# taaha-khan/2023-CompaCT-Image-Compression

Measured on AMD Instinct MI355X. Metric: MPixels/s encode+decode, 12-bit 512x512 CT batch, bytes-exact, higher is better.
Workload: dtype u16

## Files before the change

2023-compact-image-compression_amd/csrc/api.cpp:

```cpp
#include <dlfcn.h>
#include <unistd.h>
#include <zlib.h>

#include <atomic>
#include <chrono>
#include <condition_variable>
#include <functional>
#include <cstdarg>
#include <cstdio>
#include <cstdlib>
#include <cstring>
#include <map>
#include <mutex>
#include <string>
#include <thread>
#include <vector>

#include "../../include/compact_hip.h"
#include "cct_internal.h"
#include "host.h"
#include "handoff.h"

namespace cct {
bool gilbert_table(int width, int height, int32_t *out);
// ... 667 lines not shown
	dfl_bind(a, base, shape);
	a.tree_waves = (uint32_t)g_ctx.tree_waves;
	a.pos_mask = (g_ctx.compact_recs && mem_level == 8 && in_stride < ((size_t)1 << 22)) ? (1u << 22) - 1u : 0xFFFFFFFFu;
	const DevBuf &mr = E.z_ws[DFL_R_MATCH];
	if (dfl_uses_chains(strategy)) {
		if (E.z_mr_cleared != mr.p || E.z_mr_cleared_cap != mr.cap || E.z_gen_passes >= 16000u) {
			HIP_TRY(hipMemsetAsync(mr.p, 0, mr.cap, E.stream));
			HIP_TRY(hipMemsetAsync(E.z_ws[DFL_R_GEN].p, 0, 256, E.stream));
			E.z_mr_cleared = mr.p; E.z_mr_cleared_cap = mr.cap; E.z_gen_passes = 0;
		}
		E.z_gen_passes++;
	}
	a.out = (uint8_t *)E.z_out.p; a.out_stride = out_stride; a.out_sizes = (uint32_t *)E.z_outsizes.p;
	memcpy(a.header13, header13, 13);
	if (g_ctx.use_graph) {
		std::vector<uint8_t> key(sizeof(DeflateArgs) + 2 * sizeof(int));
		memcpy(key.data(), &a, sizeof(DeflateArgs));
		memcpy(key.data() + sizeof(DeflateArgs), &n, sizeof(int));
		const int fork_key = use_fork ? 1 : 0;
		memcpy(key.data() + sizeof(DeflateArgs) + sizeof(int), &fork_key, sizeof(int));
		EncSlot::ZGraph *zg = nullptr;
		for (auto &g : E.z_graphs) if (g.key == key) zg = &g;
		if (!zg) {
			const int crc = exclusive_section([&]() -> int {
				if (E.z_graphs.size() >= 4) {
					size_t old = 0;
					for (size_t i = 1; i < E.z_graphs.size(); i++) if (E.z_graphs[i].last_use < E.z_graphs[old].last_use) old = i;
					if (E.z_graphs[old].exec) (void)hipGraphExecDestroy(E.z_graphs[old].exec);
					if (E.z_graphs[old].graph) (void)hipGraphDestroy(E.z_graphs[old].graph);
					E.z_graphs.erase(E.z_graphs.begin() + (long)old);
				}
				EncSlot::ZGraph g;
				HIP_TRY(hipStreamBeginCapture(E.stream, hipStreamCaptureModeThreadLocal));
				hipError_t le = launch_deflate(a, n, E.stream, use_fork ? E.stream_side : nullptr, E.ev_fork);
				hipError_t ce = hipStreamEndCapture(E.stream, &g.graph);
				if (le != hipSuccess) { if (g.graph) (void)hipGraphDestroy(g.graph); return fail(CCT_E_DEVICE, "DEFLATE capture: %s", hipGetErrorString(le)); }
				HIP_TRY(ce);
				const hipError_t ie = hipGraphInstantiate(&g.exec, g.graph, nullptr, nullptr, 0);
				if (ie != hipSuccess) { (void)hipGraphDestroy(g.graph); return fail(CCT_E_DEVICE, "hipGraphInstantiate failed: %s", hipGetErrorString(ie)); }
				g.key = key;
				E.z_graphs.push_back(std::move(g));
				return CCT_OK;
			});
			if (crc) return crc;
			zg = &E.z_graphs.back();
		}
		zg->last_use = ++E.z_clock;
		HIP_TRY(hipGraphLaunch(zg->exec, E.stream));
		return CCT_OK;
	}
	HIP_TRY(launch_deflate(a, n, E.stream, use_fork ? E.stream_side : nullptr, E.ev_fork));
	return CCT_OK;
}

int decode_payload_locked(DecSlot &D, const uint8_t *d_payload, size_t stride, const uint32_t *d_sizes, int n, int width,
                          int height, int bs, int fractal, uint16_t *d_images, uint32_t *d_status, hipStream_t st)
{
	const int N = width * height, NB = N / bs;
	if (stride % 16 != 0) return fail(CCT_E_ARG, "payload stride must be a multiple of 16");
	if (n == 0) return CCT_OK;
	DecArgs a{};
	a.payload = d_payload; a.stride = stride; a.sizes = d_sizes;
	a.lut = nullptr;
	a.n_tiles = 0; a.n_orient = 0; a.width = width;
	if (fractal) {
		const ShapeTables *tb;
		int rc0 = get_tables(width, height, &tb);
		if (rc0) return rc0;
		a.lut = tb->d_lut;
		if (tb->tiled && g_ctx.use_tiles && !g_ctx.runtime_bs) {
			a.tile_org = tb->d_org; a.tile_orient = tb->d_orient; a.patterns = tb->d_pat;
			a.n_tiles = tb->n_tiles; a.n_orient = tb->n_orient;
		}
	}
	a.N = N; a.NB = NB; a.images = d_images; a.status = d_status;
	const size_t per = (size_t)n * NB, jper = (size_t)n * ((size_t)NB / 2 + 1);
	int rc;
	if ((rc = D.d_role.ensure(per))) return rc;
	if ((rc = D.d_slot.ensure(per * 4))) return rc;
	if ((rc = D.d_jord.ensure(jper * 4))) return rc;
	if ((rc = D.d_jval.ensure(jper))) return rc;
	a.ws_role = (uint8_t *)D.d_role.p; a.ws_slot = (uint32_t *)D.d_slot.p;
	a.ws_jord = (uint32_t *)D.d_jord.p; a.ws_jval = (uint8_t *)D.d_jval.p;
	a.pcache_steps = (int)(stride / ((size_t)g_ctx.wg_threads * DEC_SEG) + 2);
	if ((rc = D.d_pcache.ensure((size_t)n * a.pcache_steps * g_ctx.wg_threads * sizeof(uint2)))) return rc;
	a.ws_pcache = (uint2 *)D.d_pcache.p;
	const bool run_time = bs_run_time(bs, g_ctx.runtime_bs != 0);
	HIP_TRY(launch_decode(a, n, bs, g_ctx.wg_threads, st, run_time));
	g_ctx.last_dec_path = run_time ? 1 : 0;
	if (st != D.stream) {
		HIP_TRY(hipEventRecord(D.ev_ws, st));
		HIP_TRY(hipStreamWaitEvent(D.stream, D.ev_ws, 0));
	}
	return CCT_OK;
}

}
}

using namespace cct;

extern "C" {

int cct_version(void) { return CCT_ABI_VERSION; }
const char *cct_last_error(void) { return g_err; }

int cct_init(int device)
{
	std::lock_guard<std::mutex> lk(g_mu);
	return ensure_ctx(device);
}

int cct_shutdown(void)
{
	std::lock_guard<std::mutex> lk(g_mu);
	std::lock_guard<std::mutex> lk1(g_mu1);
	std::lock_guard<std::mutex> lkd0(g_mu_dec[0]);
	std::lock_guard<std::mutex> lkd1(g_mu_dec[1]);
	if (!g_ctx.ready || g_ctx.pid != getpid()) { reset_ctx(); return CCT_OK; }
	(void)hipSetDevice(g_ctx.device);
	(void)hipStreamSynchronize(g_ctx.stream);
	(void)hipStreamSynchronize(g_ctx.stream_dec);
	for (int k = 0; k < N_ENC_SLOTS; k++) {
		EncSlot &E = g_enc[k];
		if (E.stream) (void)hipStreamSynchronize(E.stream);
		if (E.stream_copy) (void)hipStreamSynchronize(E.stream_copy);
		for (auto &g : E.z_graphs) { if (g.exec) (void)hipGraphExecDestroy(g.exec); if (g.graph) (void)hipGraphDestroy(g.graph); }
		for (int i = 0; i < E.n_bufs; i++) E.all_bufs[i]->release();
		for (HandoffSet &S : E.sets) S.release();
		for (hipEvent_t e : E.ev_fork) if (e) (void)hipEventDestroy(e);
		E.ev_zlib.release();
		if (E.stream_copy) (void)hipStreamDestroy(E.stream_copy);
		if (E.stream_side) { (void)hipStreamSynchronize(E.stream_side); (void)hipStreamDestroy(E.stream_side); }
		if (k > 0 && E.stream) (void)hipStreamDestroy(E.stream);
	}
	comm_release();
	dicom_rle_release();
	jpegll_release();
	jpegls_release();
	j2k_release();
	tiff_release();
	if (g_gate) { (void)hipFree(g_gate); g_gate = nullptr; }
	for (auto &kv : g_ctx.luts) {
		ShapeTables &t = kv.second;
		void *ptrs[] = {t.d_lut, t.d_org, t.d_orient, t.d_pat, t.d_ptab, t.d_otab, t.d_ttab, t.d_htab};
		for (void *p : ptrs) if (p) (void)hipFree(p);
	}
	for (int k = 0; k < N_DEC_SLOTS; k++) {
		DecSlot &D = g_dec[k];
		if (D.stream) (void)hipStreamSynchronize(D.stream);
		D.release();
		if (k > 0 && D.stream) (void)hipStreamDestroy(D.stream);
	}
	(void)hipStreamDestroy(g_ctx.stream);
	(void)hipStreamDestroy(g_ctx.stream_dec);
	reset_ctx();
	return CCT_OK;
}

int cct_device_info(char *name, size_t name_cap, int *compute_units, uint64_t *hbm_bytes)
{
	std::lock_guard<std::mutex> lk(g_mu);
	int rc = ensure_ctx();
	if (rc) return rc;
	hipDeviceProp_t prop;
	HIP_TRY(hipGetDeviceProperties(&prop, g_ctx.device));
	if (name && name_cap) {
		char dn[256] = "";
// ... 1307 lines not shown
```

2023-compact-image-compression_amd/csrc/cct_internal.h:

```cpp
#pragma once
#include <stddef.h>
#include <stdint.h>
#include <string.h>

#include <vector>

#include <hip/hip_runtime.h>

#include "deflate_workspace.h"
#include "tuning.h"

namespace cct {

constexpr int ENC_CH = 8192;
constexpr int ENC_RING = 4;
constexpr int ENC_LIST_CAP = 1536;
constexpr int ENC_STG_BYTES = 2 * ENC_CH + ENC_CH / 8 + 64;
constexpr int ENC_MAX_LDS_ROLE = 48 * 1024;

constexpr uint8_t ROLE_PARTNER = 0xFF;

struct EncArgs {
	const uint16_t *images;
	const int32_t *lut;
	int N, NB;
	int eof;
	uint32_t flags;
	uint8_t *payload; size_t stride;
	uint32_t *sizes; uint32_t *status;
	uint8_t *ws_role;
	uint32_t *ws_lidx;
	uint64_t *ws_lmask;
	uint8_t *ws_lcur;
	uint32_t *stats;
	uint8_t *roles_out;
	uint32_t dbg_skip;
	int bs;
};
static_assert(sizeof(EncArgs) == 120, "EncArgs layout: bs must stay in the tail padding");

constexpr int TILE_MAX_TILES = 1024;
constexpr int TILE_MAX_ORIENT = 4;
struct TileEncArgs {
	EncArgs e;
	const uint32_t *tile_org;
	const uint8_t *tile_orient;
	const uint16_t *patterns;
	int n_orient, n_tiles, row_pitch;
};
size_t enc_tiles_lds_bytes(int NB, bool *role_in_lds);
hipError_t launch_encode_tiles(const TileEncArgs &ta, int n, hipStream_t s);

constexpr int STREAM_MAX_NB = 65536;
constexpr int STREAM_PAIR_REC = 80;
constexpr uint32_t CCT_ST_INTERNAL = 0x80000000u;
struct StreamTiles {
	uint32_t orgo[256];
	uint32_t last[TILE_MAX_ORIENT];
	uint32_t qorg[TILE_MAX_ORIENT];
};
constexpr int STREAM_TPG = 4;
struct StreamArgs {
	EncArgs e;
	StreamTiles tiles;
	const uint32_t *ptab;
	const uint32_t *htab;
	const uint32_t *otab;
	const uint32_t *ttab;
	int n_tiles, row_pitch, gps, tpg;
	int dbg;
	uint64_t *hand;
	uint32_t *ticket;
	uint64_t *spill_mask;
	uint16_t *spill_idx;
	uint8_t *pairrec;
};
inline size_t stream_ws_bytes(int n, int gps) { return ((size_t)n * gps * 32 + (size_t)n * 4 + 15) & ~(size_t)15; }
hipError_t launch_encode_stream(const StreamArgs &sa, int n, hipStream_t s);

size_t enc_lds_bytes(int NB, bool *role_in_lds);
inline bool bs_run_time(int bs, bool force) { return force || (bs & (bs - 1)) != 0; }

hipError_t launch_encode(const EncArgs &a, int n, int block_size, int threads, hipStream_t s, bool run_time);

constexpr int DEC_SEG = 16;
constexpr int DEC_JLIST_CAP = 2048;

struct DecArgs {
	const uint8_t *payload; size_t stride; const uint32_t *sizes;
	const int32_t *lut;
	int N, NB;
	uint16_t *images; uint32_t *status;
	uint8_t *ws_role;
	uint32_t *ws_slot;
	uint32_t *ws_jord;
	uint8_t *ws_jval;
	const uint32_t *tile_org; const uint8_t *tile_orient; const uint16_t *patterns;
	int n_tiles, n_orient, width;
	uint32_t bs_mul;
	uint2 *ws_pcache; int pcache_steps;
	uint16_t bs, bs_shift;
};
static_assert(sizeof(DecArgs) == 144, "DecArgs layout: the run-time block size fields must stay in padding");

inline void bs_divider(int d, uint32_t *mul, uint32_t *shift)
{
	uint32_t s = 0;
	while ((2u << s) <= (uint32_t)(d - 1)) s++;
	*shift = s;
	*mul = (uint32_t)((((uint64_t)1 << (32 + s)) + (uint64_t)d - 1) / (uint64_t)d);
}

hipError_t launch_decode(const DecArgs &a, int n, int block_size, int threads, hipStream_t s, bool run_time);

bool deflate_level_args(int level, DeflateArgs &a);
bool deflate_mem_level_args(int mem_level, DeflateArgs &a);
bool deflate_strategy_args(int level, int strategy, DeflateArgs &a);
hipError_t deflate_init_tables();
hipError_t launch_pack(const uint8_t *src, size_t stride, const uint32_t *sizes, int n, uint64_t *offsets, uint8_t *dst,
                       int exact, hipStream_t st);
hipError_t launch_deflate(const DeflateArgs &a, int n, hipStream_t st, hipStream_t side = nullptr,
                          const hipEvent_t *fork_join_events = nullptr);

hipError_t launch_png_filter(const uint16_t *d_img, int n, int rows, int cols, int shift, uint8_t *d_out, size_t out_stride,
                             hipStream_t st);
hipError_t launch_png_filter8(const void *d_img, int src_bits, int n, int rows, int cols, int lo, int hi, uint8_t *d_out,
                              size_t out_stride, hipStream_t st);
struct PngPackArgs {
	const uint8_t *src; size_t src_stride; uint32_t src_skip;
	const uint32_t *src_sizes;
	uint32_t chunk;
	uint8_t ihdr[25];
	uint8_t *out; size_t out_stride; uint32_t *out_sizes;
};
hipError_t launch_png_pack(const PngPackArgs &a, int n, uint32_t max_chunks, hipStream_t st);

struct PngChunk {
	uint64_t src;
	uint64_t dst;
	uint32_t len;
	uint32_t file;
};
constexpr uint32_t PNG_CHUNK_IDAT = 1u << 31;
constexpr uint32_t PNG_ST_CRC = 1u, PNG_ST_FILTER = 2u, PNG_ST_SKIP = 4u;
struct PngUnpackArgs {
	const uint8_t *files;
	const PngChunk *chunks;
	uint8_t *streams;
	uint32_t *status;
};
hipError_t launch_png_unpack(const PngUnpackArgs &a, uint32_t n_chunks, hipStream_t st);
struct PngUnfilterArgs {
	uint8_t *rows; size_t rows_stride;
	const uint32_t *row_sizes, *zstatus;
	uint32_t *status;
	const uint8_t *bpp;
	int nrows, cols, shift;
	uint16_t *images;
};
constexpr int PNG_UNFILTER_WAVES = 8;
hipError_t launch_png_unfilter(const PngUnfilterArgs &a, int n, int waves, hipStream_t st);

hipError_t launch_gate_bump(uint32_t *word, hipStream_t st);
hipError_t launch_gate_wait(const uint32_t *gate, uint32_t want_pass, uint32_t grace_us, uint32_t timeout_us, hipStream_t st);

struct InflateArgs {
	const uint8_t *in; uint64_t in_total;
	const uint64_t *offsets; int skip;
	uint8_t *out; size_t out_stride;
// ... 347 lines not shown
```

2023-compact-image-compression_amd/csrc/decode_kernels.hip:

```cpp
#include "cct_internal.h"
#include "wave_device.h"
#include "../../include/compact_hip.h"

namespace cct {
namespace {

struct SegStats {
	uint32_t exit_state;
	uint32_t npix;
	uint32_t njump;
	int32_t sdelta;
};

__device__ __forceinline__ int tok_delta_full(uint32_t b0, uint32_t b1)
{
	int x = (int)(((b0 << 8) | b1) & 0xFFFu);
	return x > 2048 ? x - 4096 : x;
}
__device__ __forceinline__ int tok_delta_short(uint32_t b0)
{
	int x = (int)(b0 & 0x7Fu);
	return x > 64 ? x - 128 : x;
}

__device__ __forceinline__ uint32_t seg_byte(const uint4 &w, uint32_t nxt, int i)
{
	const uint32_t word = (i < 4) ? w.x : (i < 8) ? w.y : (i < 12) ? w.z : (i < 16) ? w.w : nxt;
	return (word >> ((i & 3) * 8)) & 0xFFu;
}

struct SegMasks { uint32_t F, J, S, V; };

__device__ __forceinline__ uint32_t msb_nibble(uint32_t m) { return ((m >> 7) * 0x01020408u) >> 24; }

__device__ __forceinline__ SegMasks seg_masks(const uint4 &w, int nvalid)
{
	const uint32_t ws[4] = {w.x, w.y, w.z, w.w};
	SegMasks m{0, 0, 0, nvalid >= 16 ? 0xFFFFu : ((1u << max(nvalid, 0)) - 1u)};
#pragma unroll
	for (int k = 0; k < 4; k++) {
		const uint32_t x = ws[k];
		const uint32_t t = (x & 0xF0F0F0F0u) ^ 0xE0E0E0E0u;
		const uint32_t nz = (((t & 0x7F7F7F7Fu) + 0x7F7F7F7Fu) | t) & 0x80808080u;
		m.F |= msb_nibble(nz ^ 0x80808080u) << (4 * k);
		m.J |= msb_nibble(x & ~(x << 1) & 0x80808080u) << (4 * k);
		m.S |= msb_nibble(~x & 0x80808080u) << (4 * k);
	}
	m.F &= m.V; m.J &= m.V; m.S &= m.V;
	return m;
}

__device__ __forceinline__ void seg_structure(const SegMasks &m, uint32_t e, uint32_t &second, uint32_t &fulls)
{
	const uint32_t ODD = 0xAAAAAAAAu;
	const uint32_t pe = m.F & ~e;
	const uint32_t etc = (((pe << 1) | ODD) - pe) ^ ODD;
	second = (etc ^ (m.F | e)) & m.V;
	fulls = etc & m.F;
}

__device__ __forceinline__ SegStats seg_stats(const uint4 &w, uint32_t nxt, const SegMasks &m, int nvalid, uint32_t e)
{
	SegStats st{e, 0, 0, 0};
	if (nvalid <= 0) return st;
	uint32_t second, fulls;
	seg_structure(m, e, second, fulls);
	const uint32_t starts = m.V & ~second;
	st.exit_state = (fulls >> (nvalid - 1)) & 1u;
	st.njump = (uint32_t)__popc(starts & m.J);
	st.npix = (uint32_t)__popc(starts & ~m.J);
	const uint32_t sh = starts & m.S;
	const uint32_t ws[4] = {w.x, w.y, w.z, w.w};
	uint32_t sum = 0, big = 0;
#pragma unroll
	for (int k = 0; k < 4; k++) {
		const uint32_t sel = (((sh >> (4 * k)) & 15u) * 0x00204081u) & 0x01010101u;
		sum = __builtin_amdgcn_udot4(ws[k], sel, sum, false);
		big += (uint32_t)__popc(((((ws[k] & 0x7F7F7F7Fu) + 0x3F3F3F3Fu) & 0x80808080u) >> 7) & sel);
	}
	st.sdelta = (int32_t)sum - 128 * (int32_t)big;
	for (uint32_t f = fulls; f; f &= f - 1) {
		const int i = __ffs((int)f) - 1;
		st.sdelta += tok_delta_full(seg_byte(w, nxt, i), seg_byte(w, nxt, i + 1));
	}
	return st;
}

__device__ __forceinline__ uint32_t map_apply(uint32_t m, uint32_t s) { return (m >> s) & 1u; }
__device__ __forceinline__ uint32_t map_compose(uint32_t later, uint32_t earlier)
{
	return map_apply(later, map_apply(earlier, 0)) | (map_apply(later, map_apply(earlier, 1)) << 1);
}

struct Parse {
	uint32_t entry;
	uint32_t pix_base;
	int32_t val_base;
	uint32_t jump_base;
	SegStats st;
};

__device__ __forceinline__ Parse parse_step(const uint4 &w, uint32_t nxt, int nvalid,
                                           uint32_t *scratch, uint32_t &st_carry,
                                           uint32_t &npix_carry, int32_t &val_carry,
                                           uint32_t &njump_carry)
{
	const int lane = threadIdx.x & 63, wave = threadIdx.x >> 6, nw = blockDim.x >> 6;
	const SegMasks sm = seg_masks(w, nvalid);
	const SegStats s0 = seg_stats(w, nxt, sm, nvalid, 0);
	const SegStats s1 = seg_stats(w, nxt, sm, nvalid, 1);
	uint32_t m = s0.exit_state | (s1.exit_state << 1);
	m = map_compose(m, dpp_move<DPP_ROW_SHR1>(m, 2));
	m = map_compose(m, dpp_move<DPP_ROW_SHR2>(m, 2));
	m = map_compose(m, dpp_move<DPP_ROW_SHR4>(m, 2));
	m = map_compose(m, dpp_move<DPP_ROW_SHR8>(m, 2));
	m = map_compose(m, dpp_move<DPP_ROW_BCAST15, 0xA>(m, 2));
	m = map_compose(m, dpp_move<DPP_ROW_BCAST31, 0xC>(m, 2));
	const uint32_t excl = dpp_move<DPP_WAVE_SHR1>(m, 2);
	if (lane == 63) scratch[wave] = m;
	__syncthreads();
	uint32_t st_wave = st_carry, st_end = st_carry;
	for (int x = 0; x < nw; x++) {
		const uint32_t wm = scratch[x];
		if (x < wave) st_wave = map_apply(wm, st_wave);
		st_end = map_apply(wm, st_end);
	}
	Parse p;
	p.entry = map_apply(excl, st_wave);
	p.st = p.entry ? s1 : s0;
	const uint32_t ipj = wave_incl_scan(p.st.npix | (p.st.njump << 16));
	const uint32_t iv = wave_incl_scan((uint32_t)p.st.sdelta);
	const uint32_t ip = ipj & 0xFFFFu, ij = ipj >> 16;
	if (lane == 63) { scratch[16 + wave] = ipj; scratch[32 + wave] = iv; }
	__syncthreads();
	uint32_t bpj = 0, bv = 0, tpj = 0, tv = 0;
	for (int x = 0; x < nw; x++) {
		const uint32_t xp = scratch[16 + x], xv = scratch[32 + x];
		if (x < wave) { bpj += xp; bv += xv; }
		tpj += xp; tv += xv;
	}
	const uint32_t bp = bpj & 0xFFFFu, bj = bpj >> 16, tp = tpj & 0xFFFFu, tj = tpj >> 16;
	p.pix_base = npix_carry + bp + ip - p.st.npix;
	p.val_base = val_carry + (int32_t)(bv + iv - (uint32_t)p.st.sdelta);
	p.jump_base = njump_carry + bj + ij - p.st.njump;
	st_carry = st_end;
	npix_carry += tp;
	val_carry += (int32_t)tv;
	njump_carry += tj;
	return p;
}

template <int BS, bool TAB_LDS, bool TILED = false>
__global__ void __launch_bounds__(1024) decode_kernel(DecArgs a)
{
	static_assert(BS != 0 || !TILED, "the tiled variant exists for block size 16 only");
	extern __shared__ __attribute__((aligned(16))) uint8_t dyn_lds[];
	__shared__ uint32_t scratch[64];
	__shared__ uint32_t l_jord[DEC_JLIST_CAP];
	__shared__ uint8_t l_jval[DEC_JLIST_CAP];
	__shared__ uint32_t s_status;

	const int tid = threadIdx.x, T = blockDim.x;
	const int s = blockIdx.x;
	const int N = a.N, NB = a.NB;
	const uint8_t *P = a.payload + (size_t)s * a.stride;
	const uint32_t L = a.sizes[s];
	const uint32_t Lr = min((uint32_t)a.stride, L) > 0 ? min((uint32_t)a.stride, L) - 1u : 0u;
	const int32_t *lut = a.lut;
	uint16_t *out = a.images + (size_t)s * N;
	const uint32_t bs = BS ? (uint32_t)BS : (uint32_t)a.bs;
	auto bdiv = [&](uint32_t x) -> uint32_t { return BS ? x / (uint32_t)BS : __umulhi(x, a.bs_mul) >> a.bs_shift; };
	auto bmod = [&](uint32_t x) -> uint32_t { return BS ? x % (uint32_t)BS : x - bdiv(x) * bs; };
	typedef __attribute__((address_space(3))) uint8_t lds_u8;
	typedef __attribute__((address_space(3))) uint32_t lds_u32;
	lds_u32 *l_slot = (lds_u32 *)dyn_lds;
	lds_u8 *l_role = (lds_u8 *)(dyn_lds + (size_t)NB * 4);
	uint8_t *g_role = a.ws_role + (size_t)s * NB;
	uint32_t *g_slot = a.ws_slot + (size_t)s * NB;
	auto role_rd = [&](uint32_t b) -> uint32_t { return TAB_LDS ? (uint32_t)l_role[b] : (uint32_t)g_role[b]; };
	auto role_wr = [&](uint32_t b, uint32_t v) { if (TAB_LDS) l_role[b] = (uint8_t)v; else g_role[b] = (uint8_t)v; };
	auto slot_rd = [&](uint32_t i) -> uint32_t { return TAB_LDS ? l_slot[i] : g_slot[i]; };
	auto slot_wr = [&](uint32_t i, uint32_t v) { if (TAB_LDS) l_slot[i] = v; else g_slot[i] = v; };
	typedef __attribute__((address_space(3))) uint16_t lds_u16;
	constexpr uint32_t PAT_STRIDE = 4096 + 256;
	lds_u16 *l_pat = (lds_u16 *)(dyn_lds + (((size_t)NB * 5 + 15) & ~(size_t)15));
	lds_u32 *l_torg = (lds_u32 *)(l_pat + (TILED ? (size_t)a.n_orient * PAT_STRIDE : 0));
	lds_u8 *l_tori = (lds_u8 *)(l_torg + (TILED ? a.n_tiles : 0));
	if (TILED) {
		for (int i = tid; i < a.n_orient * 4096; i += T) {
			const uint32_t pv = a.patterns[i];
			const uint32_t dy = pv >> 7, dx = ((((pv >> 4) & 7u) ^ (dy & 7u)) << 3) | ((pv & 15u) >> 1);
			const uint32_t o = (uint32_t)i >> 12, p = (uint32_t)i & 4095u;
			l_pat[o * PAT_STRIDE + p + (p >> 4)] = (uint16_t)(dy * (uint32_t)a.width + dx);
		}
		for (int i = tid; i < a.n_tiles; i += T) { l_torg[i] = a.tile_org[i]; l_tori[i] = a.tile_orient[i]; }
	}
	auto raster_of = [&](uint32_t pos) -> uint32_t {
		if (TILED) {
			const uint32_t tile = pos >> 12;
			const uint32_t p = pos & 4095u;
			return l_torg[tile] + l_pat[(uint32_t)l_tori[tile] * PAT_STRIDE + p + (p >> 4)];
		}
		return lut ? (uint32_t)lut[pos] : pos;
	};
	const size_t jcap = (size_t)NB / 2 + 1;
	uint32_t *g_jord = a.ws_jord + (size_t)s * jcap;
	uint8_t *g_jval = a.ws_jval + (size_t)s * jcap;

#ifdef CCT_DEC_PROF
	long long tp[8]; int tpi = 0;
#define DEC_STAMP() do { if (tpi < 8) tp[tpi++] = clock64(); } while (0)
#else
#define DEC_STAMP() do {} while (0)
#endif
	DEC_STAMP();
	if (tid == 0) s_status = 0;
	for (int b = tid; b < NB; b += T) role_wr((uint32_t)b, 0);
	__syncthreads();
	DEC_STAMP();

	const uint32_t seg_max = (uint32_t)a.stride - 16u;
	auto load_seg = [&](uint32_t seg_start, uint4 &w, uint32_t &nxt) {
		w = *reinterpret_cast<const uint4 *>(P + min(seg_start, seg_max));
		nxt = P[min(seg_start + 16u, (uint32_t)a.stride - 1u)];
	};
	auto clip_seg = [&](uint32_t seg_start, uint4 &w, uint32_t &nxt, int &nvalid) {
		const bool inside = seg_start < Lr;
		nvalid = inside ? (int)min(16u, Lr - seg_start) : 0;
		if (!inside) w = make_uint4(0, 0, 0, 0);
		if (!(seg_start + 16u < Lr)) nxt = 0;
	};
	auto jset = [&](uint32_t k, uint32_t ord, uint32_t j) {
		if (k < DEC_JLIST_CAP) { l_jord[k] = ord; l_jval[k] = (uint8_t)j; }
		else if (k - DEC_JLIST_CAP < jcap) { g_jord[k - DEC_JLIST_CAP] = ord; g_jval[k - DEC_JLIST_CAP] = (uint8_t)j; }
	};

	uint32_t st_c = 0, npix_c = 0, nj_c = 0;
	int32_t val_c = 0;
	uint2 *pcache = a.ws_pcache + (size_t)s * a.pcache_steps * T;
	uint32_t nsteps = 0;
	uint4 wa_n; uint32_t nxta_n;
	load_seg((uint32_t)tid * DEC_SEG, wa_n, nxta_n);
	for (uint32_t base = 0; base < Lr && npix_c < (uint32_t)N; base += (uint32_t)T * DEC_SEG, nsteps++) {
		uint4 w = wa_n; uint32_t nxt = nxta_n; int nvalid;
		clip_seg(base + (uint32_t)tid * DEC_SEG, w, nxt, nvalid);
		load_seg(base + (uint32_t)(T + tid) * DEC_SEG, wa_n, nxta_n);
		const Parse p = parse_step(w, nxt, nvalid, scratch, st_c, npix_c, val_c, nj_c);
		asm volatile("" : "+v"(wa_n.x), "+v"(wa_n.y), "+v"(wa_n.z), "+v"(wa_n.w), "+v"(nxta_n) :: "memory");
		pcache[(size_t)nsteps * T + tid] = make_uint2(min(p.pix_base, 0x7FFFFFFFu) | (p.entry << 31), (uint32_t)p.val_base);
		if (p.st.njump) {
			const SegMasks sm = seg_masks(w, nvalid);
			uint32_t second, fulls;
			seg_structure(sm, p.entry, second, fulls);
			const uint32_t starts = sm.V & ~second, pix = starts & ~sm.J;
			uint32_t k = p.jump_base;
			for (uint32_t jm = starts & sm.J; jm; jm &= jm - 1, k++) {
				const int i = __ffs((int)jm) - 1;
				const uint32_t ord = p.pix_base + (uint32_t)__popc(pix & ((1u << i) - 1u));
				jset(k, ord, seg_byte(w, nxt, i) & 0x3Fu);
			}
		}
	}
	__syncthreads();
	DEC_STAMP();
	if (npix_c < (uint32_t)N && tid == 0) atomicOr(&s_status, CCT_ST_STREAM);

	if (tid < 64) {
		auto uni = [](uint32_t x) { return (uint32_t)__builtin_amdgcn_readfirstlane((int)x); };
		const uint32_t nj = uni(nj_c);
		uint32_t F = 0;
		uint64_t win = 0;
		uint32_t slots_done = 0;
		bool bad = false;
		auto fetch = [&](uint32_t k, uint32_t &ord, uint32_t &j) {
			ord = 0xFFFFFFFFu; j = 0;
			if (k < DEC_JLIST_CAP) { ord = l_jord[k]; j = l_jval[k]; }
			else if (k - DEC_JLIST_CAP < jcap) { ord = g_jord[k - DEC_JLIST_CAP]; j = g_jval[k - DEC_JLIST_CAP]; }
		};
		uint32_t ord_n = 0, j_n = 0;
		if (nj) fetch(0, ord_n, j_n);
		for (uint32_t k = 0; k < nj && !bad; k++) {
			if (k >= DEC_JLIST_CAP && k - DEC_JLIST_CAP >= jcap) { bad = true; break; }
			const uint32_t ord = uni(ord_n), j = uni(j_n);
			if (k + 1 < nj) fetch(k + 1, ord_n, j_n);
			if (ord >= (uint32_t)N) break;
			if (bmod(ord) != 0) { bad = true; break; }
			const uint32_t sslot = bdiv(ord);
			if (sslot < slots_done) { bad = true; break; }
			uint32_t remaining = sslot - slots_done;
			while (remaining) {
				if (win == 0) { F += remaining; remaining = 0; break; }
				const uint32_t o = (uint32_t)__ffsll((long long)win) - 1u;
				if (o >= remaining) { F += remaining; win >>= remaining; remaining = 0; }
				else { F += o + 1; win = (o + 1 >= 64u) ? 0ull : (win >> (o + 1)); remaining -= o; }
			}
			{ const uint64_t free_ = ~win; const uint32_t t = free_ ? (uint32_t)__builtin_ctzll(free_) : 64u; F += t; win = t >= 64u ? 0ull : win >> t; }
			const uint32_t Lb = F, pb = F + j;
			if (j == 0 || pb >= (uint32_t)NB || ((win >> j) & 1ull)) { bad = true; break; }
			if (tid == 0) { role_wr(Lb, j); role_wr(pb, ROLE_PARTNER); }
			win |= 1ull << j;
			F = Lb + 1;
			win >>= 1;
			slots_done = sslot + 2;
		}
		if (bad && tid == 0) atomicOr(&s_status, CCT_ST_STREAM);
	}
	__syncthreads();
	DEC_STAMP();

	{
		uint32_t slot_c = 0;
		for (int base = 0; base < NB; base += T) {
			const int b = base + tid;
			uint32_t r = ROLE_PARTNER, cnt = 0;
			if (b < NB) { r = role_rd((uint32_t)b); cnt = (r == ROLE_PARTNER) ? 0u : (r ? 2u : 1u); }
			const int lane = tid & 63, wave = tid >> 6, nw = T >> 6;
			const uint32_t inc = wave_incl_scan(cnt);
			if (lane == 63) scratch[wave] = inc;
			__syncthreads();
			uint32_t bs_ = 0, tot = 0;
			for (int x = 0; x < nw; x++) { const uint32_t v = scratch[x]; if (x < wave) bs_ += v; tot += v; }
			__syncthreads();
			const uint32_t sl = slot_c + bs_ + inc - cnt;
			if (cnt >= 1 && sl < (uint32_t)NB) slot_wr(sl, (uint32_t)b | (cnt == 2 ? (1u << 30) : 0u));
			if (cnt == 2 && sl + 1 < (uint32_t)NB) slot_wr(sl + 1, (uint32_t)b | (2u << 30));
			slot_c += tot;
		}
		if (slot_c != (uint32_t)NB && tid == 0) atomicOr(&s_status, CCT_ST_STREAM);
	}
	__syncthreads();
	DEC_STAMP();

	if (!(s_status & CCT_ST_STREAM)) {
		uint4 w_n; uint32_t nxt_n;
		load_seg((uint32_t)tid * DEC_SEG, w_n, nxt_n);
		uint2 pc_n = pcache[tid];
#ifdef CCT_DEC_PROF
		long long tb[4] = {0, 0, 0, 0}, tq = clock64();
#define DECB(j) do { const long long t_ = clock64(); tb[j] += t_ - tq; tq = t_; } while (0)
#else
#define DECB(j) do {} while (0)
#endif
		for (uint32_t k = 0; k < nsteps; k++) {
			const uint32_t seg_start = k * (uint32_t)T * DEC_SEG + (uint32_t)tid * DEC_SEG;
			uint4 w = w_n; uint32_t nxt = nxt_n; int nvalid;
			clip_seg(seg_start, w, nxt, nvalid);
			const uint2 pc = pc_n;
			load_seg(seg_start + (uint32_t)T * DEC_SEG, w_n, nxt_n);
			pc_n = pcache[(size_t)min(k + 1, nsteps - 1) * T + tid];
			Parse p;
			p.entry = pc.x >> 31; p.pix_base = pc.x & 0x7FFFFFFFu; p.val_base = (int32_t)pc.y;
			const SegMasks sm = seg_masks(w, nvalid);
			uint32_t second, fulls;
			seg_structure(sm, p.entry, second, fulls);
			uint32_t starts = sm.V & ~second, pix = starts & ~sm.J;
			uint32_t ord = p.pix_base;
			int32_t val = p.val_base;
			uint32_t flags = 0;
			const uint32_t room = ord < (uint32_t)N ? (uint32_t)N - ord : 0u;
			if ((uint32_t)__popc(pix) > room) {
				uint32_t keep = 0;
				if (room) {
					uint32_t pm = pix;
					for (uint32_t r = 1; r < room; r++) pm &= pm - 1;
					keep = (2u << (__ffs((int)pm) - 1)) - 1u;
				}
				starts &= keep; pix &= keep; fulls &= keep;
			}
			DECB(0);
			if (nvalid > 0 && ((fulls >> (nvalid - 1)) & 1u) && seg_start + (uint32_t)nvalid >= Lr) flags |= CCT_ST_STREAM;
			if (BS ? BS >= 16 : bs >= 16) {
				struct SlotInfo { uint32_t kind, pos0, pos1, org0, org1, idx0, idx1; };
				auto slot_info = [&](uint32_t sl) {
					SlotInfo si{0, 0, 0, 0, 0, 0, 0};
					const uint32_t ent = slot_rd(min(sl, (uint32_t)NB - 1u));
					const uint32_t blk0 = ent & 0x3FFFFFFFu; si.kind = ent >> 30;
					const uint32_t blk1 = si.kind ? blk0 + role_rd(blk0) : blk0;
					si.pos0 = blk0 * bs; si.pos1 = blk1 * bs;
					if (TILED) {
						const uint32_t t0 = si.pos0 >> 12, t1 = si.pos1 >> 12, b0 = si.pos0 & 4095u, b1 = si.pos1 & 4095u;
						si.org0 = l_torg[t0]; si.idx0 = (uint32_t)l_tori[t0] * PAT_STRIDE + b0 + (b0 >> 4);
						si.org1 = l_torg[t1]; si.idx1 = (uint32_t)l_tori[t1] * PAT_STRIDE + b1 + (b1 >> 4);
					}
					return si;
				};
				const uint32_t slA = bdiv(ord);
				const SlotInfo A = slot_info(slA), B = slot_info(slA + 1u);
				DECB(1);
				const uint32_t ws[5] = {w.x, w.y, w.z, w.w, nxt};
#pragma unroll
				for (int i = 0; i < 16; i++) {
					if (!((pix >> i) & 1u)) continue;
					const uint32_t c = (ws[i >> 2] >> (8 * (i & 3))) & 0xFFu;
					const uint32_t c1 = (ws[(i + 1) >> 2] >> (8 * ((i + 1) & 3))) & 0xFFu;
					val += ((sm.S >> i) & 1u) ? tok_delta_short(c) : ((fulls >> i) & 1u) ? tok_delta_full(c, c1) : 0;
					if ((uint32_t)val > 65535u) flags |= CCT_ST_OVERFLOW;
					const uint32_t sl = bdiv(ord), t = bmod(ord);
					const bool inA = sl == slA;
					const uint32_t kind = inA ? A.kind : B.kind;
					uint32_t odd = 0, off = t;
					if (kind) { const uint32_t mm = (kind - 1u) * bs + t; odd = mm & 1u; off = mm >> 1; }
					uint32_t ras;
					if (TILED) {
						const uint32_t org = inA ? (odd ? A.org1 : A.org0) : (odd ? B.org1 : B.org0);
						const uint32_t idx = inA ? (odd ? A.idx1 : A.idx0) : (odd ? B.idx1 : B.idx0);
						ras = org + l_pat[idx + off + (BS > 16 ? off >> 4 : 0u)];
					} else ras = raster_of((inA ? (odd ? A.pos1 : A.pos0) : (odd ? B.pos1 : B.pos0)) + off);
					out[ras] = (uint16_t)val;
					ord++;
				}
			} else {
				uint32_t cur_sl = 0xFFFFFFFFu, kind = 0, blk0 = 0, blk1 = 0;
				uint32_t org0 = 0, org1 = 0, pat0 = 0, pat1 = 0;
				for (uint32_t pm = pix; pm; pm &= pm - 1) {
					const int i = __ffs((int)pm) - 1;
					const uint32_t c = seg_byte(w, nxt, i);
					if ((sm.S >> i) & 1u) val += tok_delta_short(c);
					else if ((fulls >> i) & 1u) val += tok_delta_full(c, seg_byte(w, nxt, i + 1));
					if (val < 0 || val > 65535) flags |= CCT_ST_OVERFLOW;
					const uint32_t sl = bdiv(ord), t = bmod(ord);
					if (sl != cur_sl) {
						cur_sl = sl;
						const uint32_t ent = slot_rd(sl);
						blk0 = ent & 0x3FFFFFFFu; kind = ent >> 30;
						blk1 = kind ? blk0 + role_rd(blk0) : blk0;
						if (TILED) {
							const uint32_t t0 = (blk0 * bs) >> 12, t1 = (blk1 * bs) >> 12;
							org0 = l_torg[t0]; pat0 = (uint32_t)l_tori[t0] * PAT_STRIDE;
							org1 = l_torg[t1]; pat1 = (uint32_t)l_tori[t1] * PAT_STRIDE;
						}
					}
					uint32_t pos, odd = 0;
// ... 71 lines not shown
```

Baseline: 18410.

## Overlap jump-list replay with parsing using a dedicated wave in decode

The last wave of the decode workgroup no longer parses segments. It incrementally replays the jump list (role assignment) in chunks while the other waves parse, instead of one wave running the whole replay serially after the parse finishes. Parsing now computes only the exit-state map first and the segment stats once for the known entry state, rather than stats for both entry states. The cross-wave combines use DPP row scans and readlane instead of serial loops over scratch. The second pass is restructured to iterate over a flat segment index because the parse stride is now threads-64. The cost is one fewer parsing wave, so each workgroup needs more parse steps.

```diff
diff --git a/2023-compact-image-compression_amd/csrc/api.cpp b/2023-compact-image-compression_amd/csrc/api.cpp
--- a/2023-compact-image-compression_amd/csrc/api.cpp
+++ b/2023-compact-image-compression_amd/csrc/api.cpp
@@ -773,8 +773,9 @@
 	if ((rc = D.d_jval.ensure(jper))) return rc;
 	a.ws_role = (uint8_t *)D.d_role.p; a.ws_slot = (uint32_t *)D.d_slot.p;
 	a.ws_jord = (uint32_t *)D.d_jord.p; a.ws_jval = (uint8_t *)D.d_jval.p;
-	a.pcache_steps = (int)(stride / ((size_t)g_ctx.wg_threads * DEC_SEG) + 2);
-	if ((rc = D.d_pcache.ensure((size_t)n * a.pcache_steps * g_ctx.wg_threads * sizeof(uint2)))) return rc;
+	const size_t dec_tp = (size_t)dec_parse_lanes(g_ctx.wg_threads);
+	a.pcache_steps = (int)(stride / (dec_tp * DEC_SEG) + 2);
+	if ((rc = D.d_pcache.ensure((size_t)n * a.pcache_steps * dec_tp * sizeof(uint2)))) return rc;
 	a.ws_pcache = (uint2 *)D.d_pcache.p;
 	const bool run_time = bs_run_time(bs, g_ctx.runtime_bs != 0);
 	HIP_TRY(launch_decode(a, n, bs, g_ctx.wg_threads, st, run_time));
diff --git a/2023-compact-image-compression_amd/csrc/cct_internal.h b/2023-compact-image-compression_amd/csrc/cct_internal.h
--- a/2023-compact-image-compression_amd/csrc/cct_internal.h
+++ b/2023-compact-image-compression_amd/csrc/cct_internal.h
@@ -85,6 +85,7 @@
 
 constexpr int DEC_SEG = 16;
 constexpr int DEC_JLIST_CAP = 2048;
+constexpr int dec_parse_lanes(int threads) { return threads - 64; }
 
 struct DecArgs {
 	const uint8_t *payload; size_t stride; const uint32_t *sizes;
diff --git a/2023-compact-image-compression_amd/csrc/decode_arith.h b/2023-compact-image-compression_amd/csrc/decode_arith.h
--- /dev/null
+++ b/2023-compact-image-compression_amd/csrc/decode_arith.h
@@ -0,0 +1,140 @@
+#pragma once
+#include <stdint.h>
+
+#if defined(__HIP__)
+#include <hip/hip_runtime.h>
+#define CCT_HD __host__ __device__ __forceinline__
+#else
+#define CCT_HD inline
+#endif
+
+namespace cct {
+namespace {
+
+struct SegWords { uint32_t x, y, z, w; };
+
+CCT_HD int tok_delta_full(uint32_t b0, uint32_t b1)
+{
+	int x = (int)(((b0 << 8) | b1) & 0xFFFu);
+	return x > 2048 ? x - 4096 : x;
+}
+CCT_HD int tok_delta_short(uint32_t b0)
+{
+	int x = (int)(b0 & 0x7Fu);
+	return x > 64 ? x - 128 : x;
+}
+
+CCT_HD uint32_t seg_byte(const SegWords &w, uint32_t nxt, int i)
+{
+	const uint32_t word = (i < 4) ? w.x : (i < 8) ? w.y : (i < 12) ? w.z : (i < 16) ? w.w : nxt;
+	return (word >> ((i & 3) * 8)) & 0xFFu;
+}
+
+struct SegMasks { uint32_t F, J, S, V; };
+
+CCT_HD uint32_t msb_nibble(uint32_t m) { return ((m >> 7) * 0x01020408u) >> 24; }
+
+CCT_HD SegMasks seg_masks(const SegWords &w, int nvalid)
+{
+	const uint32_t ws[4] = {w.x, w.y, w.z, w.w};
+	SegMasks m{0, 0, 0, nvalid >= 16 ? 0xFFFFu : ((1u << (nvalid > 0 ? nvalid : 0)) - 1u)};
+#ifdef __HIP__
+#pragma unroll
+#endif
+	for (int k = 0; k < 4; k++) {
+		const uint32_t x = ws[k];
+		const uint32_t t = (x & 0xF0F0F0F0u) ^ 0xE0E0E0E0u;
+		const uint32_t nz = (((t & 0x7F7F7F7Fu) + 0x7F7F7F7Fu) | t) & 0x80808080u;
+		m.F |= msb_nibble(nz ^ 0x80808080u) << (4 * k);
+		m.J |= msb_nibble(x & ~(x << 1) & 0x80808080u) << (4 * k);
+		m.S |= msb_nibble(~x & 0x80808080u) << (4 * k);
+	}
+	m.F &= m.V; m.J &= m.V; m.S &= m.V;
+	return m;
+}
+
+CCT_HD void seg_structure(const SegMasks &m, uint32_t e, uint32_t &second, uint32_t &fulls)
+{
+	const uint32_t ODD = 0xAAAAAAAAu;
+	const uint32_t pe = m.F & ~e;
+	const uint32_t etc = (((pe << 1) | ODD) - pe) ^ ODD;
+	second = (etc ^ (m.F | e)) & m.V;
+	fulls = etc & m.F;
+}
+
+constexpr uint32_t MAP_IDENT = 2;
+CCT_HD uint32_t map_apply(uint32_t m, uint32_t s) { return (m >> s) & 1u; }
+CCT_HD uint32_t map_compose(uint32_t later, uint32_t earlier)
+{
+	return map_apply(later, map_apply(earlier, 0)) | (map_apply(later, map_apply(earlier, 1)) << 1);
+}
+
+CCT_HD uint32_t seg_exit_map(const SegMasks &m, int nvalid)
+{
+	if (nvalid <= 0) return MAP_IDENT;
+	uint32_t second, f0, f1;
+	seg_structure(m, 0, second, f0);
+	seg_structure(m, 1, second, f1);
+	return ((f0 >> (nvalid - 1)) & 1u) | (((f1 >> (nvalid - 1)) & 1u) << 1);
+}
+
+struct SegStats {
+	uint32_t exit_state;
+	uint32_t npix;
+	uint32_t njump;
+	int32_t sdelta;
+};
+
+CCT_HD uint32_t dot4_u8(uint32_t w, uint32_t sel, uint32_t acc)
+{
+#if defined(__HIP_DEVICE_COMPILE__)
+	return __builtin_amdgcn_udot4(w, sel, acc, false);
+#else
+	for (int b = 0; b < 4; b++) acc += ((w >> (8 * b)) & 0xFFu) * ((sel >> (8 * b)) & 0xFFu);
+	return acc;
+#endif
+}
+
+CCT_HD SegStats seg_stats(const SegWords &w, uint32_t nxt, const SegMasks &m, int nvalid, uint32_t e)
+{
+	SegStats st{e, 0, 0, 0};
+	if (nvalid <= 0) return st;
+	uint32_t second, fulls;
+	seg_structure(m, e, second, fulls);
+	const uint32_t starts = m.V & ~second;
+	st.exit_state = (fulls >> (nvalid - 1)) & 1u;
+	st.njump = (uint32_t)__builtin_popcount(starts & m.J);
+	st.npix = (uint32_t)__builtin_popcount(starts & ~m.J);
+	const uint32_t sh = starts & m.S;
+	const uint32_t ws[4] = {w.x, w.y, w.z, w.w};
+	uint32_t sum = 0, big = 0;
+#ifdef __HIP__
+#pragma unroll
+#endif
+	for (int k = 0; k < 4; k++) {
+		const uint32_t sel = (((sh >> (4 * k)) & 15u) * 0x00204081u) & 0x01010101u;
+		sum = dot4_u8(ws[k], sel, sum);
+		big += (uint32_t)__builtin_popcount(((((ws[k] & 0x7F7F7F7Fu) + 0x3F3F3F3Fu) & 0x80808080u) >> 7) & sel);
+	}
+	st.sdelta = (int32_t)sum - 128 * (int32_t)big;
+	for (uint32_t f = fulls; f; f &= f - 1) {
+		const int i = __builtin_ctz(f);
+		st.sdelta += tok_delta_full(seg_byte(w, nxt, i), seg_byte(w, nxt, i + 1));
+	}
+	return st;
+}
+
+CCT_HD uint32_t short_deltas4(uint32_t w)
+{
+	const uint32_t x = w & 0x7F7F7F7Fu;
+	return x | ((x + 0x3F3F3F3Fu) & 0x80808080u);
+}
+CCT_HD int32_t short_delta_at(uint32_t d4, int b) { return (int32_t)(d4 << (24 - 8 * b)) >> 24; }
+
+constexpr int COMB_LANES = 16;
+CCT_HD bool comb_lane_reads(int lane, int nw) { return lane < nw; }
+CCT_HD int comb_prefix_lane(int wave) { return wave - 1; }
+CCT_HD int comb_total_lane() { return COMB_LANES - 1; }
+
+}
+}
diff --git a/2023-compact-image-compression_amd/csrc/decode_kernels.hip b/2023-compact-image-compression_amd/csrc/decode_kernels.hip
--- a/2023-compact-image-compression_amd/csrc/decode_kernels.hip
+++ b/2023-compact-image-compression_amd/csrc/decode_kernels.hip
@@ -1,95 +1,30 @@
 #include "cct_internal.h"
 #include "wave_device.h"
+#include "decode_arith.h"
 #include "../../include/compact_hip.h"
 
 namespace cct {
 namespace {
 
-struct SegStats {
-	uint32_t exit_state;
-	uint32_t npix;
-	uint32_t njump;
-	int32_t sdelta;
-};
-
-__device__ __forceinline__ int tok_delta_full(uint32_t b0, uint32_t b1)
+#ifndef DEC_REPLAY_STEP
+#define DEC_REPLAY_STEP 8
+#endif
+
+__device__ __forceinline__ uint32_t row_scan_maps(uint32_t m)
 {
-	int x = (int)(((b0 << 8) | b1) & 0xFFFu);
-	return x > 2048 ? x - 4096 : x;
-}
-__device__ __forceinline__ int tok_delta_short(uint32_t b0)
+	m = map_compose(m, dpp_move<DPP_ROW_SHR1>(m, MAP_IDENT));
+	m = map_compose(m, dpp_move<DPP_ROW_SHR2>(m, MAP_IDENT));
+	m = map_compose(m, dpp_move<DPP_ROW_SHR4>(m, MAP_IDENT));
+	m = map_compose(m, dpp_move<DPP_ROW_SHR8>(m, MAP_IDENT));
+	return m;
+}
+__device__ __forceinline__ uint32_t row_scan_sums(uint32_t v)
 {
-	int x = (int)(b0 & 0x7Fu);
-	return x > 64 ? x - 128 : x;
-}
-
-__device__ __forceinline__ uint32_t seg_byte(const uint4 &w, uint32_t nxt, int i)
-{
-	const uint32_t word = (i < 4) ? w.x : (i < 8) ? w.y : (i < 12) ? w.z : (i < 16) ? w.w : nxt;
-	return (word >> ((i & 3) * 8)) & 0xFFu;
-}
-
-struct SegMasks { uint32_t F, J, S, V; };
-
-__device__ __forceinline__ uint32_t msb_nibble(uint32_t m) { return ((m >> 7) * 0x01020408u) >> 24; }
-
-__device__ __forceinline__ SegMasks seg_masks(const uint4 &w, int nvalid)
-{
-	const uint32_t ws[4] = {w.x, w.y, w.z, w.w};
-	SegMasks m{0, 0, 0, nvalid >= 16 ? 0xFFFFu : ((1u << max(nvalid, 0)) - 1u)};
-#pragma unroll
-	for (int k = 0; k < 4; k++) {
-		const uint32_t x = ws[k];
-		const uint32_t t = (x & 0xF0F0F0F0u) ^ 0xE0E0E0E0u;
-		const uint32_t nz = (((t & 0x7F7F7F7Fu) + 0x7F7F7F7Fu) | t) & 0x80808080u;
-		m.F |= msb_nibble(nz ^ 0x80808080u) << (4 * k);
-		m.J |= msb_nibble(x & ~(x << 1) & 0x80808080u) << (4 * k);
-		m.S |= msb_nibble(~x & 0x80808080u) << (4 * k);
-	}
-	m.F &= m.V; m.J &= m.V; m.S &= m.V;
-	return m;
-}
-
-__device__ __forceinline__ void seg_structure(const SegMasks &m, uint32_t e, uint32_t &second, uint32_t &fulls)
-{
-	const uint32_t ODD = 0xAAAAAAAAu;
-	const uint32_t pe = m.F & ~e;
-	const uint32_t etc = (((pe << 1) | ODD) - pe) ^ ODD;
-	second = (etc ^ (m.F | e)) & m.V;
-	fulls = etc & m.F;
-}
-
-__device__ __forceinline__ SegStats seg_stats(const uint4 &w, uint32_t nxt, const SegMasks &m, int nvalid, uint32_t e)
-{
-	SegStats st{e, 0, 0, 0};
-	if (nvalid <= 0) return st;
-	uint32_t second, fulls;
-	seg_structure(m, e, second, fulls);
-	const uint32_t starts = m.V & ~second;
-	st.exit_state = (fulls >> (nvalid - 1)) & 1u;
-	st.njump = (uint32_t)__popc(starts & m.J);
-	st.npix = (uint32_t)__popc(starts & ~m.J);
-	const uint32_t sh = starts & m.S;
-	const uint32_t ws[4] = {w.x, w.y, w.z, w.w};
-	uint32_t sum = 0, big = 0;
-#pragma unroll
-	for (int k = 0; k < 4; k++) {
-		const uint32_t sel = (((sh >> (4 * k)) & 15u) * 0x00204081u) & 0x01010101u;
-		sum = __builtin_amdgcn_udot4(ws[k], sel, sum, false);
-		big += (uint32_t)__popc(((((ws[k] & 0x7F7F7F7Fu) + 0x3F3F3F3Fu) & 0x80808080u) >> 7) & sel);
-	}
-	st.sdelta = (int32_t)sum - 128 * (int32_t)big;
-	for (uint32_t f = fulls; f; f &= f - 1) {
-		const int i = __ffs((int)f) - 1;
-		st.sdelta += tok_delta_full(seg_byte(w, nxt, i), seg_byte(w, nxt, i + 1));
-	}
-	return st;
-}
-
-__device__ __forceinline__ uint32_t map_apply(uint32_t m, uint32_t s) { return (m >> s) & 1u; }
-__device__ __forceinline__ uint32_t map_compose(uint32_t later, uint32_t earlier)
-{
-	return map_apply(later, map_apply(earlier, 0)) | (map_apply(later, map_apply(earlier, 1)) << 1);
+	v += dpp_move<DPP_ROW_SHR1>(v);
+	v += dpp_move<DPP_ROW_SHR2>(v);
+	v += dpp_move<DPP_ROW_SHR4>(v);
+	v += dpp_move<DPP_ROW_SHR8>(v);
+	return v;
 }
 
 struct Parse {
@@ -100,45 +35,42 @@
 	SegStats st;
 };
 
-__device__ __forceinline__ Parse parse_step(const uint4 &w, uint32_t nxt, int nvalid,
+__device__ __forceinline__ Parse parse_step(const SegWords &w, uint32_t nxt, int nvalid, bool parse,
                                            uint32_t *scratch, uint32_t &st_carry,
                                            uint32_t &npix_carry, int32_t &val_carry,
                                            uint32_t &njump_carry)
 {
-	const int lane = threadIdx.x & 63, wave = threadIdx.x >> 6, nw = blockDim.x >> 6;
-	const SegMasks sm = seg_masks(w, nvalid);
-	const SegStats s0 = seg_stats(w, nxt, sm, nvalid, 0);
-	const SegStats s1 = seg_stats(w, nxt, sm, nvalid, 1);
-	uint32_t m = s0.exit_state | (s1.exit_state << 1);
-	m = map_compose(m, dpp_move<DPP_ROW_SHR1>(m, 2));
-	m = map_compose(m, dpp_move<DPP_ROW_SHR2>(m, 2));
-	m = map_compose(m, dpp_move<DPP_ROW_SHR4>(m, 2));
-	m = map_compose(m, dpp_move<DPP_ROW_SHR8>(m, 2));
-	m = map_compose(m, dpp_move<DPP_ROW_BCAST15, 0xA>(m, 2));
-	m = map_compose(m, dpp_move<DPP_ROW_BCAST31, 0xC>(m, 2));
-	const uint32_t excl = dpp_move<DPP_WAVE_SHR1>(m, 2);
+	const int lane = threadIdx.x & 63, nw = blockDim.x >> 6;
+	const int wave = __builtin_amdgcn_readfirstlane((int)(threadIdx.x >> 6));
+	SegMasks sm{0, 0, 0, 0};
+	uint32_t m = MAP_IDENT;
+	if (parse) { sm = seg_masks(w, nvalid); m = seg_exit_map(sm, nvalid); }
+	m = row_scan_maps(m);
+	m = map_compose(m, dpp_move<DPP_ROW_BCAST15, 0xA>(m, MAP_IDENT));
+	m = map_compose(m, dpp_move<DPP_ROW_BCAST31, 0xC>(m, MAP_IDENT));
+	const uint32_t excl = dpp_move<DPP_WAVE_SHR1>(m, MAP_IDENT);
+	const bool reads = comb_lane_reads(lane, nw);
+	const int before = max(comb_prefix_lane(wave), 0);
 	if (lane == 63) scratch[wave] = m;
 	__syncthreads();
-	uint32_t st_wave = st_carry, st_end = st_carry;
-	for (int x = 0; x < nw; x++) {
-		const uint32_t wm = scratch[x];
-		if (x < wave) st_wave = map_apply(wm, st_wave);
-		st_end = map_apply(wm, st_end);
-	}
+	const uint32_t cm = row_scan_maps(reads ? scratch[lane] : MAP_IDENT);
+	const uint32_t m_before = wave ? (uint32_t)__builtin_amdgcn_readlane((int)cm, before) : MAP_IDENT;
+	const uint32_t st_wave = map_apply(m_before, st_carry);
+	const uint32_t st_end = map_apply((uint32_t)__builtin_amdgcn_readlane((int)cm, comb_total_lane()), st_carry);
 	Parse p;
 	p.entry = map_apply(excl, st_wave);
-	p.st = p.entry ? s1 : s0;
+	p.st = SegStats{p.entry, 0, 0, 0};
+	if (parse) p.st = seg_stats(w, nxt, sm, nvalid, p.entry);
 	const uint32_t ipj = wave_incl_scan(p.st.npix | (p.st.njump << 16));
 	const uint32_t iv = wave_incl_scan((uint32_t)p.st.sdelta);
 	const uint32_t ip = ipj & 0xFFFFu, ij = ipj >> 16;
 	if (lane == 63) { scratch[16 + wave] = ipj; scratch[32 + wave] = iv; }
 	__syncthreads();
-	uint32_t bpj = 0, bv = 0, tpj = 0, tv = 0;
-	for (int x = 0; x < nw; x++) {
-		const uint32_t xp = scratch[16 + x], xv = scratch[32 + x];
-		if (x < wave) { bpj += xp; bv += xv; }
-		tpj += xp; tv += xv;
-	}
+	const uint32_t cpj = row_scan_sums(reads ? scratch[16 + lane] : 0u), cv = row_scan_sums(reads ? scratch[32 + lane] : 0u);
+	const uint32_t bpj = wave ? (uint32_t)__builtin_amdgcn_readlane((int)cpj, before) : 0u;
+	const uint32_t bv = wave ? (uint32_t)__builtin_amdgcn_readlane((int)cv, before) : 0u;
+	const uint32_t tpj = (uint32_t)__builtin_amdgcn_readlane((int)cpj, comb_total_lane());
+	const uint32_t tv = (uint32_t)__builtin_amdgcn_readlane((int)cv, comb_total_lane());
 	const uint32_t bp = bpj & 0xFFFFu, bj = bpj >> 16, tp = tpj & 0xFFFFu, tj = tpj >> 16;
 	p.pix_base = npix_carry + bp + ip - p.st.npix;
 	p.val_base = val_carry + (int32_t)(bv + iv - (uint32_t)p.st.sdelta);
@@ -235,55 +167,29 @@
 		else if (k - DEC_JLIST_CAP < jcap) { g_jord[k - DEC_JLIST_CAP] = ord; g_jval[k - DEC_JLIST_CAP] = (uint8_t)j; }
 	};
 
-	uint32_t st_c = 0, npix_c = 0, nj_c = 0;
-	int32_t val_c = 0;
-	uint2 *pcache = a.ws_pcache + (size_t)s * a.pcache_steps * T;
-	uint32_t nsteps = 0;
-	uint4 wa_n; uint32_t nxta_n;
-	load_seg((uint32_t)tid * DEC_SEG, wa_n, nxta_n);
-	for (uint32_t base = 0; base < Lr && npix_c < (uint32_t)N; base += (uint32_t)T * DEC_SEG, nsteps++) {
-		uint4 w = wa_n; uint32_t nxt = nxta_n; int nvalid;
-		clip_seg(base + (uint32_t)tid * DEC_SEG, w, nxt, nvalid);
-		load_seg(base + (uint32_t)(T + tid) * DEC_SEG, wa_n, nxta_n);
-		const Parse p = parse_step(w, nxt, nvalid, scratch, st_c, npix_c, val_c, nj_c);
-		asm volatile("" : "+v"(wa_n.x), "+v"(wa_n.y), "+v"(wa_n.z), "+v"(wa_n.w), "+v"(nxta_n) :: "memory");
-		pcache[(size_t)nsteps * T + tid] = make_uint2(min(p.pix_base, 0x7FFFFFFFu) | (p.entry << 31), (uint32_t)p.val_base);
-		if (p.st.njump) {
-			const SegMasks sm = seg_masks(w, nvalid);
-			uint32_t second, fulls;
-			seg_structure(sm, p.entry, second, fulls);
-			const uint32_t starts = sm.V & ~second, pix = starts & ~sm.J;
-			uint32_t k = p.jump_base;
-			for (uint32_t jm = starts & sm.J; jm; jm &= jm - 1, k++) {
-				const int i = __ffs((int)jm) - 1;
-				const uint32_t ord = p.pix_base + (uint32_t)__popc(pix & ((1u << i) - 1u));
-				jset(k, ord, seg_byte(w, nxt, i) & 0x3Fu);
-			}
-		}
-	}
-	__syncthreads();
-	DEC_STAMP();
-	if (npix_c < (uint32_t)N && tid == 0) atomicOr(&s_status, CCT_ST_STREAM);
-
-	if (tid < 64) {
-		auto uni = [](uint32_t x) { return (uint32_t)__builtin_amdgcn_readfirstlane((int)x); };
-		const uint32_t nj = uni(nj_c);
-		uint32_t F = 0;
-		uint64_t win = 0;
-		uint32_t slots_done = 0;
-		bool bad = false;
-		auto fetch = [&](uint32_t k, uint32_t &ord, uint32_t &j) {
-			ord = 0xFFFFFFFFu; j = 0;
-			if (k < DEC_JLIST_CAP) { ord = l_jord[k]; j = l_jval[k]; }
-			else if (k - DEC_JLIST_CAP < jcap) { ord = g_jord[k - DEC_JLIST_CAP]; j = g_jval[k - DEC_JLIST_CAP]; }
-		};
+	const uint32_t Tp = (uint32_t)dec_parse_lanes(T);
+	const bool rw = __builtin_amdgcn_readfirstlane(tid >> 6) == (T >> 6) - 1;
+	auto uni = [](uint32_t x) { return (uint32_t)__builtin_amdgcn_readfirstlane((int)x); };
+	uint32_t r_F = 0, r_win_lo = 0, r_win_hi = 0, r_slots_done = 0, r_k = 0, r_end = 0;
+	auto fetch = [&](uint32_t k, uint32_t &ord, uint32_t &j) {
+		ord = 0xFFFFFFFFu; j = 0;
+		if (k < DEC_JLIST_CAP) { ord = l_jord[k]; j = l_jval[k]; }
+		else if (k - DEC_JLIST_CAP < jcap) { ord = g_jord[k - DEC_JLIST_CAP]; j = g_jval[k - DEC_JLIST_CAP]; }
+	};
+	auto replay_to = [&](uint32_t kend) {
+		if (uni(r_end) || uni(r_k) >= kend) return;
+		uint32_t F = uni(r_F);
+		uint64_t win = (uint64_t)uni(r_win_hi) << 32 | uni(r_win_lo);
+		uint32_t slots_done = uni(r_slots_done);
+		uint32_t rk = uni(r_k);
+		bool bad = false, rdone = false;
 		uint32_t ord_n = 0, j_n = 0;
-		if (nj) fetch(0, ord_n, j_n);
-		for (uint32_t k = 0; k < nj && !bad; k++) {
-			if (k >= DEC_JLIST_CAP && k - DEC_JLIST_CAP >= jcap) { bad = true; break; }
+		fetch(rk, ord_n, j_n);
+		for (; rk < kend; rk++) {
+			if (rk >= DEC_JLIST_CAP && rk - DEC_JLIST_CAP >= jcap) { bad = true; break; }
 			const uint32_t ord = uni(ord_n), j = uni(j_n);
-			if (k + 1 < nj) fetch(k + 1, ord_n, j_n);
-			if (ord >= (uint32_t)N) break;
+			if (rk + 1 < kend) fetch(rk + 1, ord_n, j_n);
+			if (ord >= (uint32_t)N) { rdone = true; break; }
 			if (bmod(ord) != 0) { bad = true; break; }
 			const uint32_t sslot = bdiv(ord);
 			if (sslot < slots_done) { bad = true; break; }
@@ -297,13 +203,56 @@
 			{ const uint64_t free_ = ~win; const uint32_t t = free_ ? (uint32_t)__builtin_ctzll(free_) : 64u; F += t; win = t >= 64u ? 0ull : win >> t; }
 			const uint32_t Lb = F, pb = F + j;
 			if (j == 0 || pb >= (uint32_t)NB || ((win >> j) & 1ull)) { bad = true; break; }
-			if (tid == 0) { role_wr(Lb, j); role_wr(pb, ROLE_PARTNER); }
+			if ((tid & 63) == 0) { role_wr(Lb, j); role_wr(pb, ROLE_PARTNER); }
 			win |= 1ull << j;
 			F = Lb + 1;
 			win >>= 1;
 			slots_done = sslot + 2;
 		}
-		if (bad && tid == 0) atomicOr(&s_status, CCT_ST_STREAM);
+		r_F = F; r_win_lo = (uint32_t)win; r_win_hi = (uint32_t)(win >> 32); r_slots_done = slots_done; r_k = rk;
+		r_end = bad ? 2u : rdone ? 1u : 0u;
+		asm volatile("" : "+v"(r_F), "+v"(r_win_lo), "+v"(r_win_hi), "+v"(r_slots_done), "+v"(r_k), "+v"(r_end));
+	};
+
+	uint32_t st_c = 0, npix_c = 0, nj_c = 0;
+	int32_t val_c = 0;
+	uint2 *pcache = a.ws_pcache + (size_t)s * a.pcache_steps * Tp;
+	uint32_t nsteps = 0;
+	uint4 wa_n; uint32_t nxta_n;
+	load_seg((uint32_t)tid * DEC_SEG, wa_n, nxta_n);
+	for (uint32_t base = 0; base < Lr && npix_c < (uint32_t)N; base += Tp * DEC_SEG, nsteps++) {
+		const uint32_t nj_before = nj_c;
+		uint4 w = wa_n; uint32_t nxt = nxta_n; int nvalid;
+		clip_seg(base + (uint32_t)tid * DEC_SEG, w, nxt, nvalid);
+		load_seg(base + (Tp + (uint32_t)tid) * DEC_SEG, wa_n, nxta_n);
+		const SegWords sw{w.x, w.y, w.z, w.w};
+		const Parse p = parse_step(sw, nxt, nvalid, !rw, scratch, st_c, npix_c, val_c, nj_c);
+		asm volatile("" : "+v"(wa_n.x), "+v"(wa_n.y), "+v"(wa_n.z), "+v"(wa_n.w), "+v"(nxta_n) :: "memory");
+		if (rw) {
+			replay_to(min(uni(nj_before), uni(r_k) + (uint32_t)DEC_REPLAY_STEP));
+		} else {
+			pcache[(size_t)nsteps * Tp + tid] = make_uint2(min(p.pix_base, 0x7FFFFFFFu) | (p.entry << 31), (uint32_t)p.val_base);
+			if (p.st.njump) {
+				const SegMasks sm = seg_masks(sw, nvalid);
+				uint32_t second, fulls;
+				seg_structure(sm, p.entry, second, fulls);
+				const uint32_t starts = sm.V & ~second, pix = starts & ~sm.J;
+				uint32_t k = p.jump_base;
+				for (uint32_t jm = starts & sm.J; jm; jm &= jm - 1, k++) {
+					const int i = __ffs((int)jm) - 1;
+					const uint32_t ord = p.pix_base + (uint32_t)__popc(pix & ((1u << i) - 1u));
+					jset(k, ord, seg_byte(sw, nxt, i) & 0x3Fu);
+				}
+			}
+		}
+	}
+	__syncthreads();
+	DEC_STAMP();
+	if (npix_c < (uint32_t)N && tid == 0) atomicOr(&s_status, CCT_ST_STREAM);
+
+	if (rw) {
+		replay_to(uni(nj_c));
+		if (r_end == 2u && (tid & 63) == 0) atomicOr(&s_status, CCT_ST_STREAM);
 	}
 	__syncthreads();
 	DEC_STAMP();
@@ -332,22 +281,25 @@
 	DEC_STAMP();
 
 	if (!(s_status & CCT_ST_STREAM)) {
+		const uint32_t nseg = nsteps * Tp, pc_last = nseg ? nseg - 1u : 0u;
 		uint4 w_n; uint32_t nxt_n;
 		load_seg((uint32_t)tid * DEC_SEG, w_n, nxt_n);
-		uint2 pc_n = pcache[tid];
+		uint2 pc_n = pcache[min((uint32_t)tid, pc_last)];
 #ifdef CCT_DEC_PROF
 		long long tb[4] = {0, 0, 0, 0}, tq = clock64();
 #define DECB(j) do { const long long t_ = clock64(); tb[j] += t_ - tq; tq = t_; } while (0)
 #else
 #define DECB(j) do {} while (0)
 #endif
-		for (uint32_t k = 0; k < nsteps; k++) {
-			const uint32_t seg_start = k * (uint32_t)T * DEC_SEG + (uint32_t)tid * DEC_SEG;
-			uint4 w = w_n; uint32_t nxt = nxt_n; int nvalid;
-			clip_seg(seg_start, w, nxt, nvalid);
-			const uint2 pc = pc_n;
+		for (uint32_t g0 = 0; g0 < nseg; g0 += (uint32_t)T) {
+			const uint32_t g = g0 + (uint32_t)tid;
+			const uint32_t seg_start = g * DEC_SEG;
+			uint4 w4 = w_n; uint32_t nxt = nxt_n; int nvalid;
+			clip_seg(g < nseg ? seg_start : Lr, w4, nxt, nvalid);
+			const uint2 pc = g < nseg ? pc_n : make_uint2(0, 0);
 			load_seg(seg_start + (uint32_t)T * DEC_SEG, w_n, nxt_n);
-			pc_n = pcache[(size_t)min(k + 1, nsteps - 1) * T + tid];
+			pc_n = pcache[min(g + (uint32_t)T, pc_last)];
+			const SegWords w{w4.x, w4.y, w4.z, w4.w};
 			Parse p;
 			p.entry = pc.x >> 31; p.pix_base = pc.x & 0x7FFFFFFFu; p.val_base = (int32_t)pc.y;
 			const SegMasks sm = seg_masks(w, nvalid);
```

After: 18560 (median of 6 runs). No clear change (+0.8%).
